# lofcz/Infidex

Hardware: AMD Instinct MI355X
Metric: queries/sec, 10M-doc corpus, top-k=20 (whole hot path, index resident in HBM) (higher is better)
Workload: dtype f32; 1 GPU; BASELINE config 4: 10000000 docs, vocab 1000000, 1 field(s), 1000-query batches, 2-3-word queries 30% fuzzed, depth 500, top-20; docs=10000000, batch=1000, top_k=20, coverage_depth=500, sessions_in_flight=4, parallelism=single GPU

## Files before the change

### infidex_amd/csrc/fused.hip.inc

```

#define P2_THREADS 256
#define P2_CAP 2048
#define P2_MAXLISTS 256
#define FQ_SKIP 1u
#define FQ_SHORT 2u
#define FQ_SHORTSKIP 4u
#define FQ_COV 8u
#define FQ_UNSUPPORTED 16u

struct FusedMeta { uint32_t s1Count, candCount; int32_t idx0, idx1; uint32_t runCov, wmAny, pad0, pad1; };

__global__ void k_rules(const infx_query* __restrict__ qs, const uint32_t* __restrict__ counts, SelRule* __restrict__ rules, uint32_t nq) {
    uint32_t i = blockIdx.x * blockDim.x + threadIdx.x;
    if (i >= nq) return;
    rules[i] = make_rule(qs[i], counts + (size_t)i * INFX_NCLASS);
}

__device__ __forceinline__ void wg_bitonic_i32(int32_t* a, uint32_t n2, int tid, int nth) {
    for (uint32_t k = 2; k <= n2; k <<= 1)
        for (uint32_t j = k >> 1; j > 0; j >>= 1) {
            for (uint32_t i = tid; i < n2; i += nth) {
                uint32_t ixj = i ^ j;
                if (ixj > i) { int32_t x = a[i], y = a[ixj]; bool up = (i & k) == 0; if (up ? (x > y) : (x < y)) { a[i] = y; a[ixj] = x; } }
            }
            __syncthreads();
        }
}
template <class Less> __device__ __forceinline__ void wg_bitonic_idx(uint16_t* idx, uint32_t n2, int tid, int nth, Less less) {
    for (uint32_t k = 2; k <= n2; k <<= 1)
        for (uint32_t j = k >> 1; j > 0; j >>= 1) {
            for (uint32_t i = tid; i < n2; i += nth) {
                uint32_t ixj = i ^ j;
                if (ixj > i) { uint16_t x = idx[i], y = idx[ixj]; bool up = (i & k) == 0; if (up ? less(y, x) : less(x, y)) { idx[i] = y; idx[ixj] = x; } }
            }
            __syncthreads();
        }
}
__device__ __forceinline__ uint32_t wg_scan_flags(const uint8_t* flag, uint32_t* pos, uint32_t n, uint32_t* part, int tid, int nth) {
    const uint32_t per = (n + nth - 1) / nth, b0 = min(n, (uint32_t)tid * per), b1 = min(n, b0 + per);
    uint32_t s = 0; for (uint32_t i = b0; i < b1; i++) s += flag[i];
    part[tid] = s; __syncthreads();
    if (tid == 0) { uint32_t run = 0; for (int i = 0; i < nth; i++) { uint32_t x = part[i]; part[i] = run; run += x; } part[nth] = run; }
    __syncthreads();
    uint32_t run = part[tid];
    for (uint32_t i = b0; i < b1; i++) { pos[i] = run; run += flag[i]; }
    const uint32_t total = part[nth];
    __syncthreads();
    return total;
}
__device__ __forceinline__ bool sorted_contains(const int32_t* a, uint32_t n, int32_t v) {
    uint32_t lo = 0, hi = n;
    while (lo < hi) { uint32_t m = (lo + hi) >> 1; if (a[m] < v) lo = m + 1; else hi = m; }
    return lo < n && a[lo] == v;
}

#ifdef SEL_PROF
__device__ unsigned long long* g_p2Prof = nullptr;
#define P2P(i) do { if (g_p2Prof && tid == 0) g_p2Prof[(size_t)qi * 8 + (i)] = wall_clock64(); } while (0)
#else
#define P2P(i)
#endif
__global__ __launch_bounds__(P2_THREADS) void k_prep2(DevIndex ix, const infx_hit* __restrict__ hits, const uint32_t* __restrict__ hitCount, int hitStride,
                                                       int W, int nd, int Dall,
                                                       const infx_fused_query* __restrict__ fqs, const infx_wm_list* __restrict__ lists,
                                                       const int32_t* __restrict__ owned, int depth, int Dp,
                                                       infx_hit* __restrict__ s1Out, infx_cov_cand* __restrict__ cands, int32_t* __restrict__ pairs, FusedMeta* __restrict__ metas) {
    extern __shared__ __attribute__((aligned(16))) unsigned char smem[];
    const uint32_t Pp = (uint32_t)max(Dp, P2_CAP);
    float* sScore = (float*)smem;
    int32_t* sDoc = (int32_t*)(sScore + Dp);
    int32_t* sTop = sDoc + Dp;
    int32_t* sUniq = sTop + Dp;
    uint32_t* sPos = (uint32_t*)(sUniq + Dp);
    int32_t* sBuf = (int32_t*)(sPos + Pp);
    long long* sKey = (long long*)(sBuf + P2_CAP);
    uint16_t* sIdx = (uint16_t*)(sKey + Dp);
    uint8_t* sFlag = (uint8_t*)(sIdx + Dp);
    unsigned long long* lBase = (unsigned long long*)(sFlag + Pp);
    uint32_t* lLen = (uint32_t*)(lBase + P2_MAXLISTS);
    uint32_t* lPos = lLen + P2_MAXLISTS;
    uint32_t* lCnt = lPos + P2_MAXLISTS;
    uint32_t* part = lCnt + P2_MAXLISTS;
    unsigned long long* sMerge = (unsigned long long*)(part + P2_THREADS + 2);
    __shared__ uint32_t shA, shB; __shared__ int32_t shT, shL0, shL1;

    const int qi = blockIdx.x, tid = threadIdx.x;
    const infx_fused_query FQ = fqs[qi];
    const uint32_t stride = 2u * (uint32_t)depth;
    infx_cov_cand* myC = cands + (size_t)qi * stride;
    FusedMeta M; M.s1Count = 0; M.candCount = 0; M.idx0 = -1; M.idx1 = -1; M.runCov = 0; M.wmAny = 0; M.pad0 = 0; M.pad1 = 0;
    int32_t* myP = pairs + (size_t)qi * stride;
    P2P(0);
    for (uint32_t i = tid; i < stride; i += P2_THREADS) { infx_cov_cand c; c.query = 0xFFFFFFFFu; c.doc = -1; c.base_score = 0.f; c.want_lcs = 0; myC[i] = c; myP[i] = -1; }
    if (FQ.flags & FQ_SKIP) { if (tid == 0) metas[qi] = M; return; }

    uint32_t c = 0;
    if (W <= 1) {
        c = FQ.dev >= 0 ? min(hitCount[FQ.dev], (uint32_t)depth) : 0u;
        for (uint32_t i = tid; i < c; i += P2_THREADS) { infx_hit h = hits[(size_t)FQ.dev * hitStride + i]; sScore[i] = h.score; sDoc[i] = h.doc; }
    } else if (FQ.dev >= 0) {
        uint32_t tot = 0;
        for (int w = 0; w < W; w++) {
            const uint32_t cw = min(hitCount[(size_t)w * nd + FQ.dev], (uint32_t)depth);
            const infx_hit* H = hits + ((size_t)w * nd + FQ.dev) * hitStride;
            for (uint32_t i = tid; i < cw; i += P2_THREADS) { const infx_hit h = H[i]; sMerge[tot + i] = ((unsigned long long)__float_as_uint(h.score) << 32) | (0xFFFFFFFFu - (uint32_t)h.doc); }
            tot += cw;
        }
        uint32_t m2 = 2; while (m2 < tot) m2 <<= 1;
        for (uint32_t i = tot + tid; i < m2; i += P2_THREADS) sMerge[i] = 0ull;
        __syncthreads();
        for (uint32_t k = 2; k <= m2; k <<= 1)
            for (uint32_t j = k >> 1; j > 0; j >>= 1) {
                for (uint32_t i = tid; i < m2; i += P2_THREADS) {
                    uint32_t ixj = i ^ j;
                    if (ixj > i) { unsigned long long a = sMerge[i], b = sMerge[ixj]; bool up = (i & k) == 0; if (up ? (a < b) : (a > b)) { sMerge[i] = b; sMerge[ixj] = a; } }
                }
                __syncthreads();
            }
        c = min(tot, (uint32_t)depth);
        for (uint32_t i = tid; i < c; i += P2_THREADS) { const unsigned long long k = sMerge[i]; sDoc[i] = (int32_t)(0xFFFFFFFFu - (uint32_t)k); sScore[i] = __uint_as_float((uint32_t)(k >> 32)); }
    }
    __syncthreads();
    for (uint32_t i = tid; i < (uint32_t)Dp; i += P2_THREADS) {
        if (i < c) sKey[i] = ix.docKeyAll[sDoc[i]];
        else { sScore[i] = -1.f; sDoc[i] = 0x7FFFFFFF; sKey[i] = 0x7FFFFFFFFFFFFFFFll; }
        sIdx[i] = (uint16_t)i;
    }
    __syncthreads();
    uint32_t c2 = 2; while (c2 < c) c2 <<= 1;
    if (c > 1) wg_bitonic_idx(sIdx, c2, tid, P2_THREADS, [&](uint16_t a, uint16_t b) {
        if (sScore[a] != sScore[b]) return sScore[a] > sScore[b];
        return sKey[a] < sKey[b]; });
    for (uint32_t i = tid; i < c; i += P2_THREADS) { uint16_t s = sIdx[i]; sTop[i] = sDoc[s]; sUniq[i] = __float_as_int(sScore[s]); }
    __syncthreads();
    for (uint32_t i = tid; i < c; i += P2_THREADS) { sDoc[i] = sTop[i]; sScore[i] = __int_as_float(sUniq[i]); }
    __syncthreads();
    for (uint32_t i = tid; i < c; i += P2_THREADS) { infx_hit h; h.doc = sDoc[i]; h.score = sScore[i]; s1Out[(size_t)qi * depth + i] = h; }
    M.s1Count = c;
    P2P(1);

    const bool isShort = (FQ.flags & FQ_SHORT) != 0;
    if ((isShort && (int)c >= FQ.max_results) || !(FQ.flags & FQ_COV) || (FQ.flags & FQ_SHORTSKIP)) { if (tid == 0) metas[qi] = M; return; }
    M.runCov = 1;

    const uint32_t nL = min(FQ.wm_count, (uint32_t)P2_MAXLISTS);
    for (uint32_t l = tid; l < nL; l += P2_THREADS) {
        const infx_wm_list L = lists[FQ.wm_off + l];
        const int32_t* p = L.src == 0 ? ix.wmExact : (L.src == 1 ? ix.wmLd1 : owned);
        lBase[l] = (unsigned long long)(uintptr_t)(p + L.off); lLen[l] = L.len; lPos[l] = 0;
    }
    M.wmAny = nL > 0 ? 1u : 0u;
    const uint32_t ntop = c;
    for (uint32_t i = tid; i < (uint32_t)Dp; i += P2_THREADS) sTop[i] = i < ntop ? sDoc[i] : 0x7FFFFFFF;
    __syncthreads();
    uint32_t t2 = 2; while (t2 < ntop) t2 <<= 1;
    if (ntop > 1) wg_bitonic_i32(sTop, t2, tid, P2_THREADS);
    P2P(2);
#ifdef SEL_PROF
    if (g_p2Prof && tid == 0) g_p2Prof[(size_t)qi * 8 + 6] = nL;
#endif
    for (uint32_t i = tid; i < ntop; i += P2_THREADS) {
        const int32_t d = sTop[i]; uint8_t f = 0;
        for (uint32_t l = 0; l < nL && !f; l++) f = sorted_contains((const int32_t*)(uintptr_t)lBase[l], lLen[l], d) ? 1 : 0;
        sFlag[i] = f;
    }
    __syncthreads();
    const uint32_t nOv = wg_scan_flags(sFlag, sPos, ntop, part, tid, P2_THREADS);
    for (uint32_t i = tid; i < ntop; i += P2_THREADS) if (sFlag[i]) { infx_cov_cand cc; cc.query = (uint32_t)qi; cc.doc = sTop[i]; cc.base_score = 0.f; cc.want_lcs = 0; myC[sPos[i]] = cc; }
    const uint32_t wmLimit = (uint32_t)max(0, depth - (int)nOv);
    const uint32_t need = max(wmLimit, 2u);
    __syncthreads();
    P2P(3);

    const uint8_t* del = q_deleted(ix, (uint32_t)nd + (uint32_t)qi);
    int32_t lv0 = -1, lv1 = -1;
    uint32_t nu = 0;
    while ((nu < need || (del && ntop + (lv0 >= 0) + (lv1 >= 0) < 2u)) && nL > 0) {
        if (tid == 0) { shA = 0; shT = 0x7FFFFFFF; shL0 = 0x7FFFFFFF; shL1 = 0x7FFFFFFF; }
        __syncthreads();
        if ((uint32_t)tid < nL && lPos[tid] < lLen[tid]) atomicAdd(&shA, 1u);
        __syncthreads();
        const uint32_t nAct = shA;
        if (nAct == 0) break;
        const uint32_t B = max(1u, (uint32_t)P2_CAP / nAct);
        if ((uint32_t)tid < nL && lPos[tid] < lLen[tid]) {
            const int32_t* p = (const int32_t*)(uintptr_t)lBase[tid];
            const uint32_t e = min(lPos[tid] + B, lLen[tid]);
            atomicMin(&shT, p[e - 1]);
        }
        __syncthreads();
        const int32_t T = shT;
        if ((uint32_t)tid < nL) {
            uint32_t cnt = 0;
            if (lPos[tid] < lLen[tid]) {
                const int32_t* p = (const int32_t*)(uintptr_t)lBase[tid];
                uint32_t lo = lPos[tid], hi = min(lPos[tid] + B, lLen[tid]);
                while (lo < hi) { uint32_t m = (lo + hi) >> 1; if (p[m] <= T) lo = m + 1; else hi = m; }
                cnt = lo - lPos[tid];
            }
            lCnt[tid] = cnt;
        }
        __syncthreads();
        if (tid == 0) { uint32_t run = 0; for (uint32_t l = 0; l < nL; l++) { uint32_t x = lCnt[l]; part[l] = run; run += x; } shB = run; }
        __syncthreads();
        const uint32_t tot = shB;
        for (uint32_t l = 0; l < nL; l++) {
            const uint32_t cnt = lCnt[l]; if (!cnt) continue;
            const int32_t* p = (const int32_t*)(uintptr_t)lBase[l] + lPos[l];
            for (uint32_t i = tid; i < cnt; i += P2_THREADS) sBuf[part[l] + i] = p[i];
        }
        __syncthreads();
        if ((uint32_t)tid < nL) lPos[tid] += lCnt[tid];
        uint32_t b2 = 2; while (b2 < tot) b2 <<= 1;
        for (uint32_t i = tot + tid; i < b2; i += P2_THREADS) sBuf[i] = 0x7FFFFFFF;
        __syncthreads();
        if (tot > 1) wg_bitonic_i32(sBuf, b2, tid, P2_THREADS);
        for (uint32_t i = tid; i < tot; i += P2_THREADS) {
            const int32_t v = sBuf[i];
            sFlag[i] = ((i == 0 || sBuf[i - 1] != v) && !sorted_contains(sTop, ntop, v)) ? 1 : 0;
        }
        __syncthreads();
        const uint32_t got = wg_scan_flags(sFlag, sPos, tot, part, tid, P2_THREADS);
        for (uint32_t i = tid; i < tot; i += P2_THREADS) if (sFlag[i] && nu + sPos[i] < need) sUniq[nu + sPos[i]] = sBuf[i];
        if (del && lv1 < 0 && ntop < 2u) {
            for (uint32_t i = tid; i < tot; i += P2_THREADS) if (sFlag[i] && !del[sBuf[i]]) atomicMin(&shL0, sBuf[i]);
            __syncthreads();
            for (uint32_t i = tid; i < tot; i += P2_THREADS) if (sFlag[i] && !del[sBuf[i]] && sBuf[i] > shL0) atomicMin(&shL1, sBuf[i]);
            __syncthreads();
            const int32_t a0 = shL0, a1 = shL1;
            if (lv0 < 0) { if (a0 != 0x7FFFFFFF) lv0 = a0; if (a1 != 0x7FFFFFFF) lv1 = a1; }
            else if (a0 != 0x7FFFFFFF) lv1 = a0;
        }
        nu = min(need, nu + got);
        __syncthreads();
    }

    P2P(4);
    int32_t f0 = -1, f1 = -1;
    { uint32_t nf = 0;
      for (uint32_t k = 0; k < ntop && nf < 2; k++) { if (nf == 0) f0 = sDoc[k]; else f1 = sDoc[k]; nf++; }
      if (!del) { for (uint32_t k = 0; k < nu && nf < 2; k++) { if (nf == 0) f0 = sUniq[k]; else f1 = sUniq[k]; nf++; } }
      else { if (nf < 2 && lv0 >= 0) { if (nf == 0) f0 = lv0; else f1 = lv0; nf++; } if (nf < 2 && lv1 >= 0) { if (nf == 0) f0 = lv1; else f1 = lv1; nf++; } } }
    M.idx0 = f0; M.idx1 = f1;
    uint32_t nWm = min(nu, wmLimit);
    for (uint32_t i = tid; i < nOv; i += P2_THREADS) { const int32_t d = myC[i].doc; if (d == f0 || d == f1) myC[i].want_lcs = 1; }
    if (!del) {
        for (uint32_t i = tid; i < nWm; i += P2_THREADS) { infx_cov_cand cc; cc.query = (uint32_t)qi; cc.doc = sUniq[i]; cc.base_score = 0.f; cc.want_lcs = (cc.doc == f0 || cc.doc == f1) ? 1 : 0; myC[nOv + i] = cc; }
    } else {
        __syncthreads();
        for (uint32_t i = tid; i < nWm; i += P2_THREADS) sFlag[i] = del[sUniq[i]] ? 0 : 1;
        __syncthreads();
        const uint32_t nLive = wg_scan_flags(sFlag, sPos, nWm, part, tid, P2_THREADS);
        for (uint32_t i = tid; i < nWm; i += P2_THREADS) if (sFlag[i]) { infx_cov_cand cc; cc.query = (uint32_t)qi; cc.doc = sUniq[i]; cc.base_score = 0.f; cc.want_lcs = (cc.doc == f0 || cc.doc == f1) ? 1 : 0; myC[nOv + sPos[i]] = cc; }
        nWm = nLive;
    }
    const float maxT = ntop ? sScore[0] : 1.f;
    for (uint32_t i = tid; i < ntop; i += P2_THREADS) {
        infx_cov_cand cc; cc.query = (uint32_t)qi; cc.doc = sDoc[i]; cc.base_score = maxT > 0.f ? sScore[i] / maxT : 0.f; cc.want_lcs = (cc.doc == f0 || cc.doc == f1) ? 1 : 0;
        myC[nOv + nWm + i] = cc;
    }
    M.candCount = nOv + nWm + ntop;
    __syncthreads();
    for (uint32_t k = tid; k < ntop && nOv > 0; k += P2_THREADS) {
        const int32_t d = sDoc[k];
        uint32_t lo = 0, hi = nOv;
        while (lo < hi) { uint32_t m = (lo + hi) >> 1; if (myC[m].doc < d) lo = m + 1; else hi = m; }
        if (lo < nOv && myC[lo].doc == d) { myP[lo] = (int32_t)((size_t)qi * stride + nOv + nWm + k); myP[nOv + nWm + k] = -2; }
    }
    __syncthreads();
    if (tid == 0) { shA = 0; shB = 0; }
    __syncthreads();
    { unsigned long long tb = 0;
      for (uint32_t i = tid; i < M.candCount; i += P2_THREADS) { const int32_t d = myC[i].doc - ix.docBase; if (d >= 0 && d < ix.N) tb += 2ull * (ix.textOff[d + 1] - ix.textOff[d]); }
      atomicAdd(&shA, (uint32_t)(tb & 0xFFFFFFFFull)); atomicAdd(&shB, (uint32_t)(tb >> 32));  }
    __syncthreads();
    if (tid == 0) { M.pad0 = shA; M.pad1 = shB; metas[qi] = M; }
    P2P(5);
}

__global__ __launch_bounds__(P2_THREADS) void k_finalize(DevIndex ix, const infx_fused_query* __restrict__ fqs, const FusedMeta* __restrict__ metas,
                                                          const infx_cov_cand* __restrict__ cands, const infx_cov_out* __restrict__ outs,
                                                          const infx_hit* __restrict__ s1, int depth, int Cp, int maxResults,
                                                          long long* __restrict__ outKeys, float* __restrict__ outScores, uint8_t* __restrict__ outTies,
                                                          uint32_t* __restrict__ outCounts, uint32_t* __restrict__ outFlags, uint32_t* __restrict__ errFlag,
                                                          int32_t* __restrict__ outDocs, const infx_finalize_setup* __restrict__ fins) {
    extern __shared__ __attribute__((aligned(16))) unsigned char smem[];
    long long* sKey = (long long*)smem;
    uint32_t* sBits = (uint32_t*)(sKey + Cp);
    uint32_t* sPos = sBits + Cp;
    uint16_t* sIdx = (uint16_t*)(sPos + Cp);
    uint8_t* sTie = (uint8_t*)(sIdx + Cp);
    uint8_t* sFlag = sTie + Cp;
    uint32_t* part = (uint32_t*)(sFlag + Cp);
    __shared__ int shMaxHits, shTrunc; __shared__ uint32_t shFirst[4], shBad;

    const int qi = blockIdx.x, tid = threadIdx.x;
    const infx_fused_query FQ = fqs[qi];
    const FusedMeta M = metas[qi];
    const int mr = min(FQ.max_results, maxResults);
    uint32_t flags = (FQ.flags & FQ_UNSUPPORTED) ? 1u : 0u;
    long long* oK = outKeys + (size_t)qi * maxResults; float* oS = outScores + (size_t)qi * maxResults; uint8_t* oT = outTies ? outTies + (size_t)qi * maxResults : nullptr;
    int32_t* oD = outDocs ? outDocs + (size_t)qi * maxResults : nullptr;
    bool useStage1 = true;
    uint32_t nOut = 0;
    if (M.runCov) {
        flags |= 2u;
        const uint32_t n = M.candCount;
        const infx_cov_cand* C = cands + (size_t)qi * 2u * depth; const infx_cov_out* O = outs + (size_t)qi * 2u * depth;
        if (tid == 0) { shMaxHits = 0; shTrunc = -1; shFirst[0] = shFirst[1] = shFirst[2] = shFirst[3] = 0xFFFFFFFFu; shBad = 0; }
        __syncthreads();
        int mh = 0;
        for (uint32_t i = tid; i < (uint32_t)Cp; i += P2_THREADS) {
            if (i < n) {
                const infx_cov_out o = O[i]; const int32_t d = C[i].doc;
                if (o.status) { atomicAdd(&shBad, 1u); atomicOr(errFlag, 1u); sKey[i] = 0x7FFFFFFFFFFFFFFFll; sBits[i] = 0; sTie[i] = 0; sIdx[i] = (uint16_t)i; continue; }
                mh = max(mh, (int)o.word_hits_full);
                sKey[i] = ix.docKeyAll[d]; sBits[i] = __float_as_uint(o.score); sTie[i] = o.tiebreaker;
                if (d == M.idx0) { if (o.word_hits) atomicMin(&shFirst[0], i); if (o.lcs) atomicMin(&shFirst[1], i); }
                if (d == M.idx1) { if (o.word_hits) atomicMin(&shFirst[2], i); if (o.lcs) atomicMin(&shFirst[3], i); }
            } else { sKey[i] = 0x7FFFFFFFFFFFFFFFll; sBits[i] = 0; sTie[i] = 0; }
            sIdx[i] = (uint16_t)i;
        }
        if (mh) atomicMax(&shMaxHits, mh);
        __syncthreads();
        const int maxWordHits = shMaxHits;
        const uint32_t nBad = shBad;
        if (nBad) flags |= 8u;
        const int hits0 = shFirst[0] != 0xFFFFFFFFu ? O[shFirst[0]].word_hits : 0, lcs0 = shFirst[1] != 0xFFFFFFFFu ? O[shFirst[1]].lcs : 0;
        const int hits1 = shFirst[2] != 0xFFFFFFFFu ? O[shFirst[2]].word_hits : 0, lcs1 = shFirst[3] != 0xFFFFFFFFu ? O[shFirst[3]].lcs : 0;
        uint32_t ncons = 0;
        if (!(maxWordHits == 0 && !M.wmAny) && n > 0) {
            uint32_t n2 = 2; while (n2 < n) n2 <<= 1;
            if (n > 1) wg_bitonic_idx(sIdx, n2, tid, P2_THREADS, [&](uint16_t a, uint16_t b) {
                const bool pa = a >= n || sKey[a] == 0x7FFFFFFFFFFFFFFFll, pb = b >= n || sKey[b] == 0x7FFFFFFFFFFFFFFFll; if (pa != pb) return pb; if (pa) return false;
                if (sBits[a] != sBits[b]) return __uint_as_float(sBits[a]) > __uint_as_float(sBits[b]);
                if (sTie[a] != sTie[b]) return sTie[a] > sTie[b];
                return sKey[a] < sKey[b]; });
            const uint32_t nf = min(n - nBad, (uint32_t)depth);
            for (uint32_t i = tid; i < nf; i += P2_THREADS) {
                const long long k = sKey[sIdx[i]]; uint8_t first = 1;
                for (uint32_t j = 0; j < i; j++) if (sKey[sIdx[j]] == k) { first = 0; break; }
                sFlag[i] = first;
            }
            __syncthreads();
            ncons = wg_scan_flags(sFlag, sPos, nf, part, tid, P2_THREADS);
            const infx_finalize_setup FS = fins[qi];
            const int minHits = max(FS.min_hits_abs, maxWordHits - FS.min_hits_relative);
            const float truncScore = (float)FS.truncation_score;
            const long long k0 = M.idx0 >= 0 ? ix.docKeyAll[M.idx0] : (long long)0x8000000000000000ull;
            const long long k1 = M.idx1 >= 0 ? ix.docKeyAll[M.idx1] : (long long)0x8000000000000000ull;
            int myTr = -1;
            for (uint32_t i = tid; i < nf; i += P2_THREADS) if (sFlag[i]) {
                const uint16_t s = sIdx[i]; int wh = 0, lc = 0;
                if (M.idx0 >= 0 && sKey[s] == k0) { wh = hits0; lc = lcs0; }
                else if (M.idx1 >= 0 && sKey[s] == k1) { wh = hits1; lc = lcs1; }
                if (wh >= minHits || lc > 0 || __uint_as_float(sBits[s]) >= truncScore) myTr = max(myTr, (int)sPos[i]);
            }
            if (myTr >= 0) atomicMax(&shTrunc, myTr);
            __syncthreads();
            const int truncIdx = FS.truncate ? shTrunc : -1;
            const int resultCount = truncIdx == -1 ? mr : min(truncIdx + 1, mr);
            ncons = min(ncons, (uint32_t)max(0, resultCount));
            if (ncons > 0) {
                useStage1 = false; nOut = min(ncons, (uint32_t)mr);
                for (uint32_t i = tid; i < nf; i += P2_THREADS) if (sFlag[i] && sPos[i] < nOut) {
                    const uint16_t s = sIdx[i]; oK[sPos[i]] = sKey[s]; oS[sPos[i]] = __uint_as_float(sBits[s]); if (oT) oT[sPos[i]] = sTie[s]; if (oD) oD[sPos[i]] = C[s].doc;
                }
            }
        }
// ... 10 lines not shown
```

### infidex_amd/csrc/infidex_hip.hip

```cpp
#include <type_traits>
#include <cstring>
#include <hip/hip_runtime.h>
#include <stdint.h>
#include <string.h>
#include <stdio.h>
#include <string>
#include <vector>
#include <unordered_map>
#include <algorithm>
#include <map>
#include <mutex>
#include <chrono>
#include <thread>
#include <dlfcn.h>
#include <rccl/rccl.h>
#include "../../include/infidex_hip.h"
#include "unicode_tables.h"

#define WAVE 64
#define FILT_MAXCOL 64

static thread_local std::string g_err;
static int32_t fail(int32_t code, const char* fmt, const char* a = "") {
    char buf[512]; snprintf(buf, sizeof buf, fmt, a); g_err = buf; return code;
// ... 1569 lines not shown
    HIPCHK(enter_device(ix->cfg.device));
    { int32_t rc_ = pin_reset(s); if (rc_) return rc_; }
    PlanStream plan(s);
    const size_t nch = word_offs[nwords];
    GROW(s->dLWordOff, s->capLWordOff, ((size_t)nwords + 1) * 4);
    GROW(s->dLChars, s->capLChars, std::max<size_t>(1, nch) * 2);
    GROW(s->dLMembers, s->capLMembers, (size_t)nwords * cap * 4);
    GROW(s->dLCount, s->capLCount, (size_t)nwords * 8);
    UP(s->dLWordOff, word_offs, ((size_t)nwords + 1) * 4);
    UP(s->dLChars, chars, nch * 2);
    uint32_t* dCnt = (uint32_t*)s->dLCount; uint32_t* dSt = dCnt + nwords;
    k_ld1<<<nwords, WAVE, 0, s->st>>>(*ix->lk, (const uint32_t*)s->dLWordOff, (const uint16_t*)s->dLChars, nwords, cap, (int32_t*)s->dLMembers, dCnt, dSt, nullptr, nullptr, 0u);
    HIPCHK(hipGetLastError());
    DOWN(counts_out, dCnt, (size_t)nwords * 4);
    DOWN(status_out, dSt, (size_t)nwords * 4);
    SYNC();
    uint32_t mx = 0; for (uint32_t i = 0; i < nwords; i++) if (!status_out[i]) mx = std::max(mx, std::min(counts_out[i], cap));
    if (mx) {
        void* p = pin_take(s, (size_t)nwords * mx * 4); if (!p) return fail(INFX_ENOMEM, "hipHostMalloc staging failed%s");
        HIPCHK(hipMemcpy2DAsync(p, (size_t)mx * 4, s->dLMembers, (size_t)cap * 4, (size_t)mx * 4, nwords, hipMemcpyDeviceToHost, s->st)); s->unsynced = true;
        SYNC();
        for (uint32_t i = 0; i < nwords; i++) { const uint32_t c = status_out[i] ? 0u : std::min(counts_out[i], cap); std::memcpy(members_out + (size_t)i * cap, (const int32_t*)p + (size_t)i * mx, (size_t)c * 4); }
    }
    return INFX_OK;
}

static std::string post_rows_text(const infx_index* ix) { return ix->postRows == INFX_FILTER_MAX_ROWS ? "INFX_FILTER_MAX_ROWS (64)" : std::to_string(ix->postRows); }
static uint32_t pow2_at_least(uint32_t v, uint32_t lo) { uint32_t p = lo; while (p < v) p <<= 1; return p; }

static uint32_t wm_words(const infx_cov_query& c) {
    uint32_t n = 0; const int nt = std::min(c.num_fusion_tokens, 2 * INFX_MAX_QUERY_TOKENS);
    for (int t = 0; t < nt; t++) if (c.ftok_len[t] >= 2 && (int)c.ftok_off[t] + (int)c.ftok_len[t] <= c.text_len) n++;
    return n;
}
static int32_t fused_check_queries(infx_index* ix, uint32_t nd, uint32_t nq, const infx_fused_query* fq, const infx_cov_query* cq,
                                   uint32_t nlists, const infx_wm_list* lists, uint32_t owned_n, int32_t depth, int32_t max_results, uint32_t nLong) {
    if (nd > nq || max_results < 1 || depth < 1 || depth > ix->cfg.max_depth) return fail(INFX_EINVAL, "bad batch shape%s");
    bool anyWm = false;
    for (uint32_t i = 0; i < nq; i++) {
        if (fq[i].dev >= (int32_t)nd) return fail(INFX_EINVAL, "fused query refers to a missing Stage-1 query%s");
        if (fq[i].wm_count > INFX_MAX_WM_LISTS || (uint64_t)fq[i].wm_off + fq[i].wm_count > nlists) return fail(INFX_ECAPACITY, "too many WordMatcher lists for one query%s");
        if (fq[i].wm_count) anyWm = true;
        if (fq[i].flags & INFX_FQ_BROWSE) {
            if (!(fq[i].flags & INFX_FQ_SKIP) || (fq[i].flags & INFX_FQ_UNSUPPORTED)) return fail(INFX_EINVAL, "INFX_FQ_BROWSE goes with INFX_FQ_SKIP: a browse query has no text%s");
            if (fq[i].max_results > (int32_t)ix->postRows) return fail(INFX_EUNSUPPORTED, "a browse query returns at most %s rows (its facets run on them; infx_set_post_rows)", post_rows_text(ix).c_str());
        }
        if (fq[i].flags & INFX_FQ_WMDEV) {
            if (!ix->haveDict) return fail(INFX_EINVAL, "INFX_FQ_WMDEV needs infx_upload_wm_dictionary%s");
            if (fq[i].wm_count) return fail(INFX_EINVAL, "a query takes its WordMatcher lists either from the caller or from the device lookup%s");
            if ((fq[i].flags & INFX_FQ_COV) && !(fq[i].flags & INFX_FQ_SKIP) && wm_words(cq[i]) * (uint32_t)(3 + 2 * ix->lk->maxLd1) > INFX_MAX_WM_LISTS)
                return fail(INFX_ECAPACITY, "too many words for the device WordMatcher lookup (hand the lists over instead)%s");
        }
        if ((fq[i].flags & INFX_FQ_COV) && !(fq[i].flags & INFX_FQ_SKIP) && cq[i].reserved != 0) {
            if (cq[i].reserved < 0 || (uint32_t)cq[i].reserved > nLong) return fail(INFX_EINVAL, "query refers to a missing long-query record (infx_stage2_long_queries)%s");
            if (fq[i].flags & INFX_FQ_WMDEV) return fail(INFX_EINVAL, "the device WordMatcher lookup reads the words of a fast-envelope query: hand the lists of a long query over%s");
        } else if ((fq[i].flags & INFX_FQ_COV) && !(fq[i].flags & INFX_FQ_SKIP) &&
            (cq[i].num_tokens > INFX_MAX_QUERY_TOKENS || cq[i].text_len > INFX_MAX_QUERY_CHARS || cq[i].num_fusion_tokens > 2 * INFX_MAX_QUERY_TOKENS))
            return fail(INFX_EUNSUPPORTED, "query exceeds the Stage-2 envelope (hand it over as a long query: infx_stage2_long_queries)%s");
    }
    for (uint32_t l = 0; l < nlists; l++) {
        const infx_wm_list& L = lists[l];
        const uint64_t lim = L.src == 0 ? ix->nWmExact : (L.src == 1 ? ix->nWmLd1 : (L.src == 2 ? owned_n : 0));
        if (L.off + L.len > lim) return fail(INFX_EINVAL, "WordMatcher list out of range%s");
    }
    if (anyWm && !ix->haveWm) return fail(INFX_EINVAL, "infx_upload_wordmatcher has not been called%s");
    return INFX_OK;
}

static int32_t fused_enqueue_select(infx_stream* s, uint32_t nd, int32_t depth, bool shardNext = false, bool markTurn = false) {
    infx_index* ix = s->ix;
    GROW(s->dRules, s->capRules, std::max<size_t>(1, nd) * sizeof(SelRule));
    GROW(s->dHits, s->capHits, std::max<size_t>(1, (size_t)nd) * depth * sizeof(infx_hit));
    GROW(s->dHitCount, s->capHitCount, std::max<size_t>(1, nd) * 4);
    GROW(s->dFQueries, s->capFQueries, std::max<size_t>(1, nd) * sizeof(infx_query));
    UP(s->dFQueries, s->lastQ.data(), (size_t)nd * sizeof(infx_query));
    HIPCHK(hipMemsetAsync(s->dHitCount, 0, std::max<size_t>(1, nd) * 4, s->st));
    Arena ar = make_arena(s);
    HIPCHK(hipEventRecord(s->evS0, s->st));
    if (nd) {
        k_rules<<<(nd + 255) / 256, 256, 0, s->st>>>((const infx_query*)s->dFQueries, (const uint32_t*)s->dCounts, (SelRule*)s->dRules, nd);
        const bool exact = !shardNext && exact_possible(s);
        if (exact) HIPCHK(hipMemsetAsync(s->dExactStat + 4, 0, 16, s->st));
        if (shardNext) GROW(s->dNext, s->capNext, (size_t)nd * 4);
#ifdef SEL_PROF
        static unsigned long long* dProf = nullptr; static int profCalls = 0;
        if (getenv("INFX_SEL_PROF") && nd >= 500) { if (!dProf) { hipMalloc((void**)&dProf, 4096 * 64); hipMemcpyToSymbol(HIP_SYMBOL(g_selProf), &dProf, sizeof(dProf)); } hipMemsetAsync(dProf, 0, (size_t)nd * 64, s->st); }
#endif
        const uint32_t* selOrd = select_order(s, nd);
        const SelGiant selG = select_giants(s, ar, nd, selOrd);
        k_select<<<nd, SEL_THREADS, 0, s->st>>>(ar, ix->d.nRanges, (const SelRule*)s->dRules, (infx_hit*)s->dHits, (uint32_t*)s->dHitCount, depth, exact ? (uint32_t*)s->dExactFlag : nullptr, exact ? s->dExactStat + 4 : nullptr,
                                                shardNext ? (float*)s->dNext : nullptr, selOrd, selG);
#ifdef SEL_PROF
        if (dProf && nd >= 500 && ++profCalls == 6) { static const char* const ph[5] = {"hist1", "hist2", "gather", "sort", "write"}; wgprof_dump("selprof", dProf, nd, ph, s->st); }
#endif
        if (markTurn) { HIPCHK(hipEventRecord(s->evTurn, s->st)); markTurn = false; }
        if (exact) { int32_t rc_ = mark_wide_queries(s, ix->cfg.max_depth); if (rc_) return rc_; }
        if (exact) { int32_t rc_ = enqueue_exact(s, nd, depth); if (rc_) return rc_; }
    }
    if (markTurn) HIPCHK(hipEventRecord(s->evTurn, s->st));
    HIPCHK(hipGetLastError());
    HIPCHK(hipEventRecord(s->evS1, s->st));
    s->timedSel = true;
    return INFX_OK;
}

static int32_t fused_enqueue_prep_stage2(infx_stream* s, int W, uint32_t nd, const infx_hit* dHitsAll, const uint32_t* dHcAll,
                                         uint32_t nq, const infx_fused_query* fq, const infx_cov_query* cq, uint32_t nlists, const infx_wm_list* lists,
                                         uint32_t owned_n, const int32_t* owned, int32_t depth, int32_t want_debug) {
    infx_index* ix = s->ix;
    const uint32_t stride = 2u * (uint32_t)depth, ncand = nq * stride;
    const uint32_t Dp = pow2_at_least((uint32_t)depth, 8);
    const uint32_t Dall = W > 1 ? pow2_at_least((uint32_t)W * (uint32_t)depth, 8) : 0;
    if (Dall > 8192) return fail(INFX_ECAPACITY, "shards x depth exceeds the in-LDS merge (8192 rows); merge hierarchically%s");
    s->browseQ.clear();
    for (uint32_t i = 0; i < nq; i++) if (fq[i].flags & INFX_FQ_BROWSE) s->browseQ.push_back({i, (uint32_t)std::max(fq[i].max_results, 0)});
    s->qpRows.clear();
    if (ix->postRows > INFX_FILTER_MAX_ROWS) { s->qpRows.resize(nq); for (uint32_t i = 0; i < nq; i++) s->qpRows[i] = fq[i].max_results; }
    GROW(s->dFQ, s->capFQ, (size_t)nq * sizeof(infx_fused_query));
    GROW(s->dFLists, s->capFLists, std::max<size_t>(1, nlists) * sizeof(infx_wm_list));
    GROW(s->dFOwned, s->capFOwned, ((size_t)owned_n + 1) * 4);
    GROW(s->dFS1, s->capFS1, (size_t)nq * depth * sizeof(infx_hit));
    GROW(s->dFMeta, s->capFMeta, (size_t)nq * sizeof(FusedMeta));
    GROW(s->dCovQ, s->capCovQ, (size_t)nq * sizeof(infx_cov_query));
    GROW(s->dCovC, s->capCovC, (size_t)ncand * sizeof(infx_cov_cand));
    GROW(s->dCovO, s->capCovO, (size_t)ncand * sizeof(infx_cov_out));
    GROW(s->dFPairs, s->capFPairs, (size_t)ncand * 4);
    if (want_debug) GROW(s->dCovF, s->capCovF, (size_t)ncand * INFX_NFEAT * 4);
    std::vector<infx_fused_query> fqDev; uint64_t wmSlots = 0;
    for (uint32_t i = 0; i < nq; i++) if (fq[i].flags & INFX_FQ_WMDEV) {
        if (fqDev.empty()) fqDev.assign(fq, fq + nq);
        fqDev[i].reserved = (int32_t)wmSlots;
        if ((fq[i].flags & INFX_FQ_COV) && !(fq[i].flags & INFX_FQ_SKIP)) wmSlots += wm_words(cq[i]);
    }
    const bool wmDev = !fqDev.empty();
    if (wmDev) {
        if (wmSlots * WM_AFFIX_CAP + owned_n > 0x7FFFFFF0ull) return fail(INFX_ECAPACITY, "device WordMatcher lookup: too many query words in one batch%s");
        GROW(s->dFLists, s->capFLists, ((size_t)nlists + (size_t)nq * INFX_MAX_WM_LISTS) * sizeof(infx_wm_list));
        GROW(s->dFOwned, s->capFOwned, ((size_t)owned_n + (size_t)wmSlots * WM_AFFIX_CAP + 1) * 4);
    }
    UP(s->dFQ, wmDev ? fqDev.data() : fq, (size_t)nq * sizeof(infx_fused_query));
    UP(s->dFLists, lists, (size_t)nlists * sizeof(infx_wm_list));
    UP(s->dFOwned, owned, (size_t)owned_n * 4);
    UP(s->dCovQ, cq, (size_t)nq * sizeof(infx_cov_query));
    s->batchAlias = s->longAlias;
    for (uint32_t i = 0; i < nq && !s->batchAlias; i++) if (cq[i].reserved == 0) for (int32_t k = 0; k < cq[i].text_len && k < (int32_t)INFX_MAX_QUERY_CHARS; k++) if (s2_host_is_alias(cq[i].text[k])) { s->batchAlias = true; break; }
    HIPCHK(hipMemsetAsync(s->dCovO, 0, (size_t)ncand * sizeof(infx_cov_out), s->st));
    HIPCHK(hipEventRecord(s->evP0, s->st));
    if (wmDev) {
        DevLookup lk = *ix->lk; if (s->csOn && !s->cs.cover_prefix_suffix) lk.nAffix = 0;
        k_wm<<<nq, WAVE, 0, s->st>>>(lk, (infx_fused_query*)s->dFQ, (const infx_cov_query*)s->dCovQ, nq, (infx_wm_list*)s->dFLists, nlists, (int32_t*)s->dFOwned, (uint64_t)owned_n);
        HIPCHK(hipGetLastError());
    }
    {
        const size_t Pp = std::max<size_t>(Dp, P2_CAP);
        const size_t lds = (size_t)Dp * 4 * 4 + Pp * 4 + (size_t)P2_CAP * 4 + (size_t)Dp * 8 + (size_t)Dp * 2 + Pp + (size_t)P2_MAXLISTS * (8 + 4 + 4 + 4) + (P2_THREADS + 2) * 4 + (size_t)Dall * 8 + 64;
        if (lds > 64 * 1024) HIPCHK(hipFuncSetAttribute((const void*)k_prep2, hipFuncAttributeMaxDynamicSharedMemorySize, (int)lds));
#ifdef SEL_PROF
        static unsigned long long* dP2 = nullptr; static int p2Calls = 0;
        if (getenv("INFX_SEL_PROF") && nq >= 500) { if (!dP2) { hipMalloc((void**)&dP2, 4096 * 64); hipMemcpyToSymbol(HIP_SYMBOL(g_p2Prof), &dP2, sizeof(dP2)); } hipMemsetAsync(dP2, 0, (size_t)nq * 64, s->st); }
#endif
        k_prep2<<<nq, P2_THREADS, lds, s->st>>>(dev_index(s), dHitsAll, dHcAll, depth, W, (int)nd, (int)Dall, (const infx_fused_query*)s->dFQ,
                                                 (const infx_wm_list*)s->dFLists, (const int32_t*)s->dFOwned, depth, (int)Dp,
                                                 (infx_hit*)s->dFS1, (infx_cov_cand*)s->dCovC, (int32_t*)s->dFPairs, (FusedMeta*)s->dFMeta);
#ifdef SEL_PROF
        if (dP2 && nq >= 500 && ++p2Calls == 6) { static const char* const ph[5] = {"s1sort", "topsort", "overlap", "wmrounds", "emit"}; wgprof_dump("p2prof", dP2, nq, ph, s->st); }
#endif
    }
    HIPCHK(hipGetLastError());
    HIPCHK(hipEventRecord(s->evP1, s->st));
    HIPCHK(hipEventRecord(s->evC0, s->st));
    S2_LAUNCH_FAST(dev_index(s), (const infx_cov_query*)s->dCovQ, nq, (const infx_cov_cand*)s->dCovC, ncand,
                                                                                 (infx_cov_out*)s->dCovO, want_debug ? (int32_t*)s->dCovF : nullptr, 1, 0, (const int32_t*)s->dFPairs);
    S2_LAUNCH_SLOW(dev_index(s), (const infx_cov_query*)s->dCovQ, nq, (const infx_cov_cand*)s->dCovC, ncand,
                                                                                 (infx_cov_out*)s->dCovO, want_debug ? (int32_t*)s->dCovF : nullptr, 1, 1, (const int32_t*)s->dFPairs);
    { int32_t rc_ = s2_huge_ready(s); if (rc_) return rc_; }
    S2_LAUNCH_HUGE(dev_index(s), (const infx_cov_query*)s->dCovQ, nq, (const infx_cov_cand*)s->dCovC, ncand,
                                                                                 (infx_cov_out*)s->dCovO, want_debug ? (int32_t*)s->dCovF : nullptr, 1, 1, (const int32_t*)s->dFPairs);
    S2_LAUNCH_LONGQ(dev_index(s), (const infx_cov_query*)s->dCovQ, nq, (const infx_cov_cand*)s->dCovC, ncand,
                                                                                 (infx_cov_out*)s->dCovO, want_debug ? (int32_t*)s->dCovF : nullptr, 1, 1, (const int32_t*)s->dFPairs);
    HIPCHK(hipGetLastError());
    HIPCHK(hipEventRecord(s->evC1, s->st));
    s->timedCov = true;
    s->fusedNq = nq; s->fusedDepth = depth; s->fusedDebug = want_debug != 0;
    return INFX_OK;
}

#define FCM_MAXK 4096u
#define FCM_MAXGRID 2048
static int32_t count_enqueue(infx_stream* s, const DevFilter* dProgs, uint32_t K, const DevCountCols& cc, int32_t docBase, int32_t n, uint32_t* dCounts) {
    infx_index* ix = s->ix;
    { int32_t rc_ = columns_cover(ix, (int64_t)docBase + std::max(n, 0), COLS_COVER_COUNTED); if (rc_) return rc_; }
    HIPCHK(hipMemsetAsync(dCounts, 0, (size_t)K * 4, s->st));
    s->lastCountK = K; s->lastCountLaunches = 0;
    if (n <= 0 || !K) return INFX_OK;
    const DevColumns cols = dev_columns(ix);
    const int grid = (int)std::min<int64_t>(FCM_MAXGRID, ((int64_t)n + FCM_THREADS - 1) / FCM_THREADS);
    for (uint32_t k0 = 0; k0 < K; k0 += FCM_MAXK) {
        const uint32_t k = std::min(FCM_MAXK, K - k0);
        const size_t lds = ((size_t)k + (size_t)cc.nUsed * FCM_THREADS) * 4;
        HIPCHK(lds_limit((const void*)k_filter_count_multi, ix->cfg.device, lds));
        k_filter_count_multi<<<grid, FCM_THREADS, lds, s->st>>>(dProgs + k0, k, cc, cols, docBase, n, ix->d.deleted, dCounts + k0);
        HIPCHK(hipGetLastError());
        s->lastCountLaunches++;
    }
    return INFX_OK;
}

static int mask_slot_of(const infx_stream* s, const uint8_t* p) { for (int i = 0; i < INFX_MAX_PREFILTERS; i++) if (p && s->dMask[i] == p) return i; return -1; }
static inline size_t mask_bytes(const infx_index* ix) { return (((size_t)std::max(ix->d.totalDocs, 0) + 3) & ~(size_t)3) + 4; }
static int32_t mask_flush(infx_stream* s) {
    if (!s->mkStaged) return INFX_OK;
    s->mkStaged = false;
    infx_index* ix = s->ix;
    const uint32_t K = s->mkTable.size();
    const int32_t n = ix->d.totalDocs;
    s->lastMaskBuilt = K; s->lastMaskLaunches = 0;
    if (!K) return INFX_OK;
    { int32_t rc_ = columns_cover(ix, n, COLS_COVER_CORPUS); if (rc_) return rc_; }
    for (uint32_t k = 0; k < K; k++) {
        const int slot = mask_slot_of(s, s->mkOut.mask[k]);
        if (slot < 0 || s->capMask[slot] < mask_bytes(ix)) return fail(INFX_EINVAL, "a mask buffer is not a mask slot of this stream, or was made for a smaller corpus%s");
    }
    { int32_t rc_ = table_upload(s, s->mkTable, &s->dMaskBlob, &s->capMaskBlob); if (rc_) return rc_; }
    GROW(s->dMaskCnt, s->capMaskCnt, (size_t)INFX_MAX_PREFILTERS * 4);
    HIPCHK(hipMemsetAsync(s->dMaskCnt, 0, (size_t)K * 4, s->st));
    if (n > 0) {
        const DevColumns cols = dev_columns(ix);
        const DevCountCols cc = s->mkTable.columns(0, K);
        const int threads = ((size_t)cc.nUsed * 4 * FMM_THREADS + K) * 4 <= 40 * 1024 ? FMM_THREADS : WAVE;
        const size_t lds = ((size_t)cc.nUsed * 4 * threads + K) * 4;
        const int64_t groups = ((int64_t)n + 3) / 4;
        const int grid = (int)std::min<int64_t>(FCM_MAXGRID, (groups + threads - 1) / threads);
        HIPCHK(lds_limit((const void*)k_filter_mask_multi, ix->cfg.device, lds));
        k_filter_mask_multi<<<grid, threads, lds, s->st>>>((const DevFilter*)s->dMaskBlob, K, cc, cols, n, ix->d.deleted, s->mkOut, (uint32_t*)s->dMaskCnt);
        HIPCHK(hipGetLastError());
        s->lastMaskLaunches = 1;
    }
    if (s->mkCountsOut) DOWN(s->mkCountsOut, s->dMaskCnt, (size_t)K * 4);
    return INFX_OK;
}
static int32_t stage_doc_masks(infx_stream* s, uint32_t nd, uint32_t nq, const infx_fused_query* fq) {
    s->qDelOn = false;
    bool any = false; for (auto m : s->docMasks) any = any || m != nullptr;
    if (!any) return INFX_OK;
    infx_index* ix = s->ix;
    std::vector<const uint8_t*> tbl((size_t)nd + nq, ix->d.deleted); std::vector<uint8_t> set(nd, 0);
    for (uint32_t i = 0; i < nq; i++) {
        const uint8_t* m = s->docMasks[i] ? s->docMasks[i] : ix->d.deleted;
        if (s->docMasks[i]) { const int slot = mask_slot_of(s, m); if (slot < 0 || s->capMask[slot] < mask_bytes(ix)) return fail(INFX_EINVAL, "a document mask is not a mask slot of this stream, or was made for a smaller corpus%s"); }
        tbl[(size_t)nd + i] = m;
        const int32_t d = fq[i].dev;
        if (d < 0 || (uint32_t)d >= nd) continue;
        if (set[d] && tbl[d] != m) return fail(INFX_EINVAL, "two queries with different document masks share one Stage-1 query%s");
        tbl[d] = m; set[d] = 1;
    }
    GROW(s->dQDel, s->capQDel, tbl.size() * sizeof(const uint8_t*));
    UP(s->dQDel, tbl.data(), tbl.size() * sizeof(const uint8_t*));
    s->qDelOn = true;
    return INFX_OK;
}

#define BRW_MAXG 256u
#define BRW_MAXRANGES 2048
static int32_t browse_enqueue(infx_stream* s, const ProgTable& T, const char* dCode, const DevQPost* desc, uint32_t descStride, uint32_t ncount, int32_t max_results, bool ties) {
    infx_index* ix = s->ix;
    const int32_t n = ix->d.totalDocs;
    { int32_t rc_ = columns_cover(ix, n, COLS_COVER_CORPUS); if (rc_) return rc_; }
    static const bool earlyStop = [] { const char* e = getenv("INFX_BROWSE_EARLY_STOP"); return !(e && e[0] == '0'); }();
    const uint32_t rowStride = ix->postRows;
    std::vector<DevBrowseGroup> groups; std::vector<DevBrowseQuery> bq; std::unordered_map<int32_t, uint32_t> groupOf;
    for (auto& b : s->browseQ) {
        const int32_t prog = desc[(size_t)b.first * descStride].filter;
        auto it = groupOf.find(prog);
        if (it == groupOf.end()) { it = groupOf.emplace(prog, (uint32_t)groups.size()).first; groups.push_back(DevBrowseGroup{prog >= 0 ? T.dev((uint32_t)prog, dCode) : DevFilter{}, prog, 0u, 0u, 0u}); }
        const uint32_t rows = std::min<uint32_t>(std::min<uint32_t>(b.second, (uint32_t)max_results), rowStride);
        groups[it->second].rows = std::max(groups[it->second].rows, rows);
        bq.push_back(DevBrowseQuery{b.first, it->second, rows, 0u});
    }
    for (uint32_t k = 0; k < ncount; k++) {
        auto it = groupOf.find((int32_t)k);
        if (it == groupOf.end()) { it = groupOf.emplace((int32_t)k, (uint32_t)groups.size()).first; groups.push_back(DevBrowseGroup{T.dev(k, dCode), (int32_t)k, 0u, 0u, 0u}); }
        groups[it->second].flags |= BRW_COUNT; groups[it->second].countIdx = k;
    }
    const uint32_t G = (uint32_t)groups.size();
    const int64_t tiles = ((int64_t)std::max(n, 1) + BRW_THREADS - 1) / BRW_THREADS;
    const uint32_t nRanges = (uint32_t)std::min<int64_t>(BRW_MAXRANGES, tiles);
    const bool dup = ix->firstLive != nullptr;
    auto al = [](size_t x) { return (x + 15) & ~(size_t)15; };
    const size_t oBq = al((size_t)G * sizeof(DevBrowseGroup)), blob = oBq + bq.size() * sizeof(DevBrowseQuery);
    const size_t oPre = al((size_t)G * nRanges * 4), oTot = oPre + oPre, oOwn = oTot + al((size_t)G * 4), oRows = oOwn + al((size_t)G * 4), work = oRows + (size_t)G * rowStride * 4;
    GROW(s->dBrwBlob, s->capBrwBlob, blob); GROW(s->dBrwWork, s->capBrwWork, work);
    std::vector<uint8_t> H(blob, 0);
    std::memcpy(H.data(), groups.data(), (size_t)G * sizeof(DevBrowseGroup)); std::memcpy(H.data() + oBq, bq.data(), bq.size() * sizeof(DevBrowseQuery));
    UP(s->dBrwBlob, H.data(), blob);
    const DevBrowseGroup* dGroups = (const DevBrowseGroup*)s->dBrwBlob; const DevBrowseQuery* dBq = (const DevBrowseQuery*)((char*)s->dBrwBlob + oBq);
    char* W = (char*)s->dBrwWork;
    uint32_t *dCnt = (uint32_t*)W, *dPre = (uint32_t*)(W + oPre), *dTot = (uint32_t*)(W + oTot), *dOwn = (uint32_t*)(W + oOwn); int32_t* dRows = (int32_t*)(W + oRows);
    if (ncount) { GROW(s->dQCount, s->capQCount, (size_t)ncount * 4); HIPCHK(hipMemsetAsync(s->dQCount, 0, (size_t)ncount * 4, s->st)); }
    if (dup) HIPCHK(hipMemsetAsync(dOwn, 0, (size_t)G * 4, s->st));
    const DevColumns cols = dev_columns(ix);
    s->lastBrowseGroups = G; s->lastBrowseLaunches = 0;
    for (uint32_t g0 = 0; g0 < G; g0 += BRW_MAXG) {
        const uint32_t g = std::min(BRW_MAXG, G - g0);
        DevCountCols cc{};
        for (uint32_t i = 0; i < g; i++) if (groups[g0 + i].prog >= 0) T.add_columns(cc, (uint32_t)groups[g0 + i].prog);
        const size_t lds = ((size_t)g * (dup ? 2 : 1) + (size_t)cc.nUsed * BRW_THREADS * (dup ? 2 : 1)) * 4;
        if (dup) {
            HIPCHK(lds_limit((const void*)k_browse_scan<true>, ix->cfg.device, lds));
            k_browse_scan<true><<<nRanges, BRW_THREADS, lds, s->st>>>(dGroups + g0, g, cc, cols, n, (uint32_t)tiles, nRanges, ix->d.deleted, ix->firstLive, earlyStop ? 1 : 0,
                                                                       dCnt + (size_t)g0 * nRanges, dOwn + g0);
        } else {
            HIPCHK(lds_limit((const void*)k_browse_scan<false>, ix->cfg.device, lds));
            k_browse_scan<false><<<nRanges, BRW_THREADS, lds, s->st>>>(dGroups + g0, g, cc, cols, n, (uint32_t)tiles, nRanges, ix->d.deleted, nullptr, earlyStop ? 1 : 0,
                                                                        dCnt + (size_t)g0 * nRanges, nullptr);
        }
        HIPCHK(hipGetLastError());
        s->lastBrowseLaunches++;
    }
// ... 1221 lines not shown
```

Baseline: 94490 queries/s.

## Rework k_prep2 overlap and word-match merge with sampled search and merge-path

Templates k_prep2 on a NEW flag, enabled by default, with the old path kept behind INFX_PREP2_REF. The new path skips the stage-1 bitonic sort when the candidates are already in order. It tests overlap with per-pair binary search over LDS-cached samples of each word-match list, then a short global search. It replaces the bitonic sort of gathered list chunks with a parallel merge-path tree merge of the already-sorted runs. It also aliases scratch LDS regions to shrink the per-workgroup footprint, which risks aliasing bugs and adds index arithmetic.

```diff
diff --git a/infidex_amd/csrc/fused.hip.inc b/infidex_amd/csrc/fused.hip.inc
--- a/infidex_amd/csrc/fused.hip.inc
+++ b/infidex_amd/csrc/fused.hip.inc
@@ -53,6 +53,21 @@
     while (lo < hi) { uint32_t m = (lo + hi) >> 1; if (a[m] < v) lo = m + 1; else hi = m; }
     return lo < n && a[lo] == v;
 }
+__device__ __forceinline__ bool sorted_contains_g(gint32p a, uint32_t n, int32_t v) {
+    uint32_t lo = 0, hi = n;
+    while (lo < hi) { uint32_t m = (lo + hi) >> 1; if (a[m] < v) lo = m + 1; else hi = m; }
+    return lo < n && a[lo] == v;
+}
+__device__ __forceinline__ uint32_t p2_samp_step(uint32_t len, uint32_t ns) { return ns == len ? 1u : (len - 1 + ns - 2) / (ns - 1); }
+__device__ __forceinline__ uint32_t p2_samp_pos(uint32_t j, uint32_t step, uint32_t len) { return min(j * step, len - 1); }
+__host__ __device__ constexpr uint32_t p2_scratch_bytes(bool NEW, uint32_t Dp, uint32_t Pp) {
+    return NEW ? (Pp * 4 + P2_CAP * 4 > Dp * 10 ? Pp * 4 + P2_CAP * 4 : Dp * 10) : Pp * 4 + P2_CAP * 4 + Dp * 10;
+}
+__host__ __device__ constexpr size_t p2_lds_bytes(bool NEW, uint32_t Dp, uint32_t Dall) {
+    const uint32_t Pp = Dp > P2_CAP ? Dp : P2_CAP;
+    return (size_t)Dp * 16 + p2_scratch_bytes(NEW, Dp, Pp) + Pp + (size_t)P2_MAXLISTS * (NEW ? 16 : 20) + (P2_THREADS + 2) * 4 + (size_t)Dall * 8 + (NEW ? 0 : 64);
+}
+static_assert(P2_CAP == 8 * P2_THREADS, "the merge rounds of k_prep2 give every thread eight consecutive output slots");
 
 #ifdef SEL_PROF
 __device__ unsigned long long* g_p2Prof = nullptr;
@@ -60,6 +75,7 @@
 #else
 #define P2P(i)
 #endif
+template <int NEW>
 __global__ __launch_bounds__(P2_THREADS) void k_prep2(DevIndex ix, const infx_hit* __restrict__ hits, const uint32_t* __restrict__ hitCount, int hitStride,
                                                        int W, int nd, int Dall,
                                                        const infx_fused_query* __restrict__ fqs, const infx_wm_list* __restrict__ lists,
@@ -73,14 +89,14 @@
     int32_t* sUniq = sTop + Dp;
     uint32_t* sPos = (uint32_t*)(sUniq + Dp);
     int32_t* sBuf = (int32_t*)(sPos + Pp);
-    long long* sKey = (long long*)(sBuf + P2_CAP);
+    long long* sKey = NEW ? (long long*)sPos : (long long*)(sBuf + P2_CAP);
     uint16_t* sIdx = (uint16_t*)(sKey + Dp);
-    uint8_t* sFlag = (uint8_t*)(sIdx + Dp);
+    uint8_t* sFlag = (uint8_t*)sPos + p2_scratch_bytes(NEW, (uint32_t)Dp, Pp);
     unsigned long long* lBase = (unsigned long long*)(sFlag + Pp);
     uint32_t* lLen = (uint32_t*)(lBase + P2_MAXLISTS);
     uint32_t* lPos = lLen + P2_MAXLISTS;
     uint32_t* lCnt = lPos + P2_MAXLISTS;
-    uint32_t* part = lCnt + P2_MAXLISTS;
+    uint32_t* part = NEW ? lCnt : lCnt + P2_MAXLISTS;
     unsigned long long* sMerge = (unsigned long long*)(part + P2_THREADS + 2);
     __shared__ uint32_t shA, shB; __shared__ int32_t shT, shL0, shL1;
 
@@ -128,6 +144,14 @@
     }
     __syncthreads();
     uint32_t c2 = 2; while (c2 < c) c2 <<= 1;
+    int unsorted = 1;
+    if (NEW) {
+        unsorted = 0;
+        for (uint32_t i = tid; i + 1 < c; i += P2_THREADS)
+            if (!(sScore[i] > sScore[i + 1] || (sScore[i] == sScore[i + 1] && sKey[i] < sKey[i + 1]))) unsorted = 1;
+        unsorted = __syncthreads_or(unsorted);
+    }
+    if (unsorted) {
     if (c > 1) wg_bitonic_idx(sIdx, c2, tid, P2_THREADS, [&](uint16_t a, uint16_t b) {
         if (sScore[a] != sScore[b]) return sScore[a] > sScore[b];
         return sKey[a] < sKey[b]; });
@@ -135,6 +159,7 @@
     __syncthreads();
     for (uint32_t i = tid; i < c; i += P2_THREADS) { sDoc[i] = sTop[i]; sScore[i] = __int_as_float(sUniq[i]); }
     __syncthreads();
+    }
     for (uint32_t i = tid; i < c; i += P2_THREADS) { infx_hit h; h.doc = sDoc[i]; h.score = sScore[i]; s1Out[(size_t)qi * depth + i] = h; }
     M.s1Count = c;
     P2P(1);
@@ -159,10 +184,40 @@
 #ifdef SEL_PROF
     if (g_p2Prof && tid == 0) g_p2Prof[(size_t)qi * 8 + 6] = nL;
 #endif
+    if (!NEW) {
     for (uint32_t i = tid; i < ntop; i += P2_THREADS) {
         const int32_t d = sTop[i]; uint8_t f = 0;
         for (uint32_t l = 0; l < nL && !f; l++) f = sorted_contains((const int32_t*)(uintptr_t)lBase[l], lLen[l], d) ? 1 : 0;
         sFlag[i] = f;
+    }
+    } else {
+        int32_t* sSamp = (int32_t*)sPos;
+        const uint32_t share = nL ? (Pp + P2_CAP) / nL : 0u;
+        for (uint32_t g = tid; g < nL * share; g += P2_THREADS) {
+            const uint32_t l = g / share, j = g - l * share, len = lLen[l], ns = min(len, share);
+            if (j < ns) sSamp[g] = ((gint32p)lBase[l])[p2_samp_pos(j, p2_samp_step(len, ns), len)];
+        }
+        for (uint32_t i = tid; i < ntop; i += P2_THREADS) sFlag[i] = 0;
+        __syncthreads();
+        volatile uint8_t* vFlag = sFlag;
+        const uint32_t npair = ntop * nL;
+        for (uint32_t p = tid; p < npair; p += P2_THREADS) {
+            const uint32_t l = p / ntop, i = p - l * ntop;
+            if (vFlag[i]) continue;
+            const int32_t d = sTop[i];
+            const uint32_t len = lLen[l], ns = min(len, share);
+            const int32_t* sm = sSamp + l * share;
+            if (!ns || d < sm[0] || d > sm[ns - 1]) continue;
+            uint32_t lo = 0, hi = ns;
+            while (lo < hi) { uint32_t m = (lo + hi) >> 1; if (sm[m] <= d) lo = m + 1; else hi = m; }
+            const uint32_t j = lo - 1;
+            bool f = sm[j] == d;
+            if (!f && ns < len) {
+                const uint32_t step = p2_samp_step(len, ns), a = p2_samp_pos(j, step, len) + 1, b = p2_samp_pos(j + 1, step, len);
+                f = sorted_contains_g((gint32p)lBase[l] + a, b - a, d);
+            }
+            if (f) vFlag[i] = 1;
+        }
     }
     __syncthreads();
     const uint32_t nOv = wg_scan_flags(sFlag, sPos, ntop, part, tid, P2_THREADS);
@@ -198,12 +253,46 @@
                 while (lo < hi) { uint32_t m = (lo + hi) >> 1; if (p[m] <= T) lo = m + 1; else hi = m; }
                 cnt = lo - lPos[tid];
             }
-            lCnt[tid] = cnt;
-        }
-        __syncthreads();
-        if (tid == 0) { uint32_t run = 0; for (uint32_t l = 0; l < nL; l++) { uint32_t x = lCnt[l]; part[l] = run; run += x; } shB = run; }
+            if (NEW) part[tid] = cnt; else lCnt[tid] = cnt;
+        }
+        __syncthreads();
+        if (tid == 0) { uint32_t run = 0; for (uint32_t l = 0; l < nL; l++) { uint32_t x = NEW ? part[l] : lCnt[l]; part[l] = run; run += x; } if (NEW) part[nL] = run; shB = run; }
         __syncthreads();
         const uint32_t tot = shB;
+        if (NEW) {
+            uint32_t nlev = 0; while ((1u << nlev) < nL) nlev++;
+            int32_t* src = (nlev & 1) ? (int32_t*)sPos : sBuf;
+            int32_t* dst = (nlev & 1) ? sBuf : (int32_t*)sPos;
+            for (uint32_t e = tid; e < tot; e += P2_THREADS) {
+                uint32_t lo = 0, hi = nL;
+                while (lo < hi) { uint32_t m = (lo + hi) >> 1; if (part[m] <= e) lo = m + 1; else hi = m; }
+                const uint32_t l = lo - 1;
+                src[e] = ((gint32p)lBase[l])[lPos[l] + (e - part[l])];
+            }
+            __syncthreads();
+            if ((uint32_t)tid < nL) lPos[tid] += part[tid + 1] - part[tid];
+            for (uint32_t s = 0; s < nlev; s++) {
+                const uint32_t npr = (nL + (2u << s) - 1) >> (s + 1);
+                uint32_t o = (uint32_t)tid * 8u; const uint32_t oEnd = min(tot, o + 8u);
+                while (o < oEnd) {
+                    uint32_t lo = 0, hi = npr;
+                    while (lo < hi) { uint32_t m = (lo + hi) >> 1; if (part[min(m << (s + 1), nL)] <= o) lo = m + 1; else hi = m; }
+                    const uint32_t q = lo - 1;
+                    const uint32_t a0 = part[min(q << (s + 1), nL)], b0 = part[min((2 * q + 1) << s, nL)], b1 = part[min((q + 1) << (s + 1), nL)];
+                    const uint32_t d = o - a0, la = b0 - a0, lb = b1 - b0;
+                    uint32_t x = d > lb ? d - lb : 0u, y = min(d, la);
+                    while (x < y) { uint32_t m = (x + y) >> 1; if (src[a0 + m] <= src[b0 + d - 1 - m]) x = m + 1; else y = m; }
+                    uint32_t ia = a0 + x, ib = b0 + (d - x);
+                    int32_t va = ia < b0 ? src[ia] : 0, vb = ib < b1 ? src[ib] : 0;
+                    for (const uint32_t stop = min(oEnd, b1); o < stop; o++) {
+                        if (ib >= b1 || (ia < b0 && va <= vb)) { dst[o] = va; if (++ia < b0) va = src[ia]; }
+                        else { dst[o] = vb; if (++ib < b1) vb = src[ib]; }
+                    }
+                }
+                __syncthreads();
+                int32_t* t = src; src = dst; dst = t;
+            }
+        } else {
         for (uint32_t l = 0; l < nL; l++) {
             const uint32_t cnt = lCnt[l]; if (!cnt) continue;
             const int32_t* p = (const int32_t*)(uintptr_t)lBase[l] + lPos[l];
@@ -215,6 +304,7 @@
         for (uint32_t i = tot + tid; i < b2; i += P2_THREADS) sBuf[i] = 0x7FFFFFFF;
         __syncthreads();
         if (tot > 1) wg_bitonic_i32(sBuf, b2, tid, P2_THREADS);
+        }
         for (uint32_t i = tid; i < tot; i += P2_THREADS) {
             const int32_t v = sBuf[i];
             sFlag[i] = ((i == 0 || sBuf[i - 1] != v) && !sorted_contains(sTop, ntop, v)) ? 1 : 0;
diff --git a/infidex_amd/csrc/infidex_hip.hip b/infidex_amd/csrc/infidex_hip.hip
--- a/infidex_amd/csrc/infidex_hip.hip
+++ b/infidex_amd/csrc/infidex_hip.hip
@@ -1745,18 +1745,19 @@
         HIPCHK(hipGetLastError());
     }
     {
-        const size_t Pp = std::max<size_t>(Dp, P2_CAP);
-        const size_t lds = (size_t)Dp * 4 * 4 + Pp * 4 + (size_t)P2_CAP * 4 + (size_t)Dp * 8 + (size_t)Dp * 2 + Pp + (size_t)P2_MAXLISTS * (8 + 4 + 4 + 4) + (P2_THREADS + 2) * 4 + (size_t)Dall * 8 + 64;
-        if (lds > 64 * 1024) HIPCHK(hipFuncSetAttribute((const void*)k_prep2, hipFuncAttributeMaxDynamicSharedMemorySize, (int)lds));
+        static const bool ref = [] { const char* e = getenv("INFX_PREP2_REF"); return e && e[0] == '1'; }();
+        const auto kern = ref ? k_prep2<0> : k_prep2<1>;
+        const size_t lds = p2_lds_bytes(!ref, Dp, Dall);
+        if (lds > 64 * 1024) HIPCHK(hipFuncSetAttribute((const void*)kern, hipFuncAttributeMaxDynamicSharedMemorySize, (int)lds));
 #ifdef SEL_PROF
         static unsigned long long* dP2 = nullptr; static int p2Calls = 0;
         if (getenv("INFX_SEL_PROF") && nq >= 500) { if (!dP2) { hipMalloc((void**)&dP2, 4096 * 64); hipMemcpyToSymbol(HIP_SYMBOL(g_p2Prof), &dP2, sizeof(dP2)); } hipMemsetAsync(dP2, 0, (size_t)nq * 64, s->st); }
 #endif
-        k_prep2<<<nq, P2_THREADS, lds, s->st>>>(dev_index(s), dHitsAll, dHcAll, depth, W, (int)nd, (int)Dall, (const infx_fused_query*)s->dFQ,
-                                                 (const infx_wm_list*)s->dFLists, (const int32_t*)s->dFOwned, depth, (int)Dp,
-                                                 (infx_hit*)s->dFS1, (infx_cov_cand*)s->dCovC, (int32_t*)s->dFPairs, (FusedMeta*)s->dFMeta);
+        kern<<<nq, P2_THREADS, lds, s->st>>>(dev_index(s), dHitsAll, dHcAll, depth, W, (int)nd, (int)Dall, (const infx_fused_query*)s->dFQ,
+                                              (const infx_wm_list*)s->dFLists, (const int32_t*)s->dFOwned, depth, (int)Dp,
+                                              (infx_hit*)s->dFS1, (infx_cov_cand*)s->dCovC, (int32_t*)s->dFPairs, (FusedMeta*)s->dFMeta);
 #ifdef SEL_PROF
-        if (dP2 && nq >= 500 && ++p2Calls == 6) { static const char* const ph[5] = {"s1sort", "topsort", "overlap", "wmrounds", "emit"}; wgprof_dump("p2prof", dP2, nq, ph, s->st); }
+        if (dP2 && nq >= 500 && ++p2Calls == 6) { fprintf(stderr, "[p2prof] %s, %zu B of dynamic LDS per workgroup\n", ref ? "k_prep2<0> (INFX_PREP2_REF)" : "k_prep2<1>", lds); static const char* const ph[5] = {"s1sort", "topsort", "overlap", "wmrounds", "emit"}; wgprof_dump("p2prof", dP2, nq, ph, s->st); }
 #endif
     }
     HIPCHK(hipGetLastError());
```

After: 87780 queries/s. 0.929x the previous value.
